# felipefelixarias/a2cat-vn-pytorch

Hardware: AMD Instinct MI355X
Metric: env-steps/sec (whole node), 4096 parallel cached-THOR envs at 1/2/4/8 GPUs (higher is better)
Workload: dtype u8; 1 GPU; cached-THOR VectorEnv.step, 20 synthetic 24x24 scenes (626 MB frame cache, HBM-resident), 4096 envs/GPU, 84x84x3 frames, uniform random actions, auto-reset, TimeLimit 900; envs_per_gpu=4096, scenes=20, parallelism=dp1 (independent env shards, replicated scene cache)

## Files before the change

a2cat-vn-pytorch_amd/csrc/vn_policy.hip:

```cpp
#include <hip/hip_runtime.h>

#include <algorithm>
#include <cstdio>
#include <cstdlib>
#include <mutex>
#include <new>
#include <map>
#include <tuple>
#include <unordered_map>

#include "vn_common.h"
#include "vn_gemm.h"
#include "vn_lstm.h"
#include "vn_aux.h"
#include "vn_unreal.h"
#include "vn_skinny.h"

#include "vn_frames.h"
#include "vn_conv1.h"
namespace vn {

template <int H, int W, int OH, int OW>
struct FramesIm2col {
  FrameSrc src;
// ... 932 lines not shown
  DgradA<COUT, 4, 2, OH, OW, HYC, WXC> fa{dz, M};
  DgradB<COUT, 4, 2, CINF> fb{WT, cin, g * cin, PY, PX};
  EpiMaskParity<H, W, 2, PY, PX, HYC, WXC> ep{out, X, g, G, cin};
  launch_gemm_x6<128, 32, 32, 4, 1>(fa, fb, ep, M, cin, 4 * COUT, st);
}

template <int H, int OH>
constexpr int k4s2_covered() {
  return H < 2 * (OH - 1) + 4 ? H : 2 * (OH - 1) + 4;
}

template <int H, int W, int CH, int CW>
__global__ void zero_uncovered_kernel(float* __restrict__ out, int nimg_g, int cin) {
  constexpr int NU = H * W - CH * CW;
  const int64_t i = (int64_t)blockIdx.x * blockDim.x + threadIdx.x;
  const int c4n = cin / 4;
  if (i >= (int64_t)nimg_g * NU * c4n) return;
  const int c4 = (int)(i % c4n);
  const int64_t q = i / c4n;
  const int u = (int)(q % NU);
  const int64_t ng = q / NU;
  int y, x;
  if (u < (H - CH) * W) {
    y = CH + u / W;
    x = u % W;
  } else {
    const int v = u - (H - CH) * W;
    y = v / (W - CW);
    x = CW + v % (W - CW);
  }
  *reinterpret_cast<f4*>(out + ((ng * H + y) * W + x) * cin + 4 * c4) = f4zero();
}

template <int SH_, int SW_, int YC_, int XC_, int KC_, int NCOL_, int WPC_>
struct ParityDg {
  static constexpr int SH = SH_, SW = SW_, YC = YC_, XC = XC_, KC = KC_, NCOL = NCOL_, WPC = WPC_;
  static constexpr int NP = SH * SW;
  static constexpr int NPC = YC * XC;
  static constexpr int PS = KC + 8;
  static constexpr int rows(int img) { return (img * NPC + 15) / 16 * 16 + XC + 1; }
  static constexpr int IMG = NPC >= 64 ? ((size_t)3 * rows(2) * KC * 2 <= 160 * 1024 ? 2 : 1) : 64 / NPC;
  static constexpr int NR = rows(IMG);
  static constexpr int NTL = NCOL / (16 * WPC);
  static constexpr int KS = KC / 32;
  static constexpr int NT = 256 * WPC;
  static constexpr size_t LDS = (size_t)3 * NR * KC * 2;
  static constexpr bool fits = LDS <= 160 * 1024;
  static_assert(KC % 32 == 0 && NCOL % (16 * WPC) == 0, "k steps of 32, whole 16-column tiles per wave");
  static_assert(KC == 32 || KC == 64, "plane rows of 4 or 8 quads (dg_quad_off)");
  static_assert(XC == SW + 1 && YC == SH + 1, "k4 s2 classes: the map plus one gap row and column");
};

template <class S, class EP>
__global__ __launch_bounds__(S::NT, S::NT >= 512 ? 1 : 2) void parity_dgrad_x6_kernel(const float* __restrict__ map,
                                                                const float* __restrict__ WT, EP ep, int n) {
  constexpr int SW = S::SW, XC = S::XC, KC = S::KC, NCOL = S::NCOL, WPC = S::WPC;
  constexpr int NP = S::NP, NPC = S::NPC, IMG = S::IMG, NTL = S::NTL, KS = S::KS, NT = S::NT;
  constexpr int ROWS = IMG * NP, PL = S::NR * KC, C4 = KC / 4, NQ = KC / 8;
  constexpr int TILES = (IMG * NPC + 15) / 16, NZ = (ROWS * C4 + NT - 1) / NT;
  extern __shared__ __attribute__((aligned(16))) uint8_t smem_pdg[];
  uint16_t* zs = reinterpret_cast<uint16_t*>(smem_pdg);
  const int tid = threadIdx.x, lane = tid & 63;
  const int wave = __builtin_amdgcn_readfirstlane(tid >> 6);
  const int cls = wave / WPC, py = cls >> 1, px = cls & 1;
  const int col0 = (wave % WPC) * NTL * 16;
  const int i16 = lane & 15, q = lane >> 4;
  bf16x8_t bw[4][KS][NTL][3];
#pragma unroll
  for (int t = 0; t < 4; ++t) {
    const int ky = py + 2 * (t >> 1), kx = px + 2 * (t & 1);
#pragma unroll
    for (int h = 0; h < KS; ++h)
#pragma unroll
      for (int nt = 0; nt < NTL; ++nt) {
        union { uint16_t u[8]; bf16x8_t v; } b0, b1, b2;
        const float* w = WT + ((int64_t)(ky * 4 + kx) * NCOL + col0 + 16 * nt + i16) * KC + 32 * h + 8 * q;
#pragma unroll
        for (int j = 0; j < 8; ++j) split3_bf16(w[j], b0.u[j], b1.u[j], b2.u[j]);
        bw[t][h][nt][0] = b0.v;
        bw[t][h][nt][1] = b1.v;
        bw[t][h][nt][2] = b2.v;
      }
  }
  for (int i = tid; i < 3 * PL / 8; i += NT) reinterpret_cast<uint4*>(zs)[i] = uint4{0u, 0u, 0u, 0u};
  __syncthreads();
  const int items = (n + IMG - 1) / IMG;
  f4 zr[NZ];
  auto load_z = [&](int it) {
    const int64_t r0 = (int64_t)it * ROWS, rend = (int64_t)n * NP;
    const f4* z4 = reinterpret_cast<const f4*>(map);
#pragma unroll
    for (int j = 0; j < NZ; ++j) {
      const int i = tid + j * NT;
      if (i < ROWS * C4) zr[j] = r0 + i / C4 < rend ? z4[(r0 + i / C4) * C4 + i % C4] : f4zero();
    }
  };
  constexpr bool PF = NZ <= 3;
  if (PF && (int)blockIdx.x < items) load_z(blockIdx.x);
  for (int it = blockIdx.x; it < items; it += gridDim.x) {
    if constexpr (!PF) load_z(it);
#pragma unroll
    for (int j = 0; j < NZ; ++j) {
      const int i = tid + j * NT;
      if (i < ROWS * C4) {
        uint2 t0, t1, t2;
        split3_pack(zr[j], t0, t1, t2);
        const int pix = i / C4, c = i - (i / C4) * C4, im = pix / NP, rem = pix - (pix / NP) * NP;
        const int row = im * NPC + (rem / SW + 1) * XC + rem % SW + 1;
        uint16_t* d = zs + dg_quad_off<NQ>(row, c >> 1) + 4 * (c & 1);
// ... 32 lines not shown
            c = __builtin_amdgcn_mfma_f32_16x16x32_bf16(bw[tap][h][nt][2], a[0], c, 0, 0, 0);
            c = __builtin_amdgcn_mfma_f32_16x16x32_bf16(bw[tap][h][nt][1], a[1], c, 0, 0, 0);
            c = __builtin_amdgcn_mfma_f32_16x16x32_bf16(bw[tap][h][nt][0], a[1], c, 0, 0, 0);
            c = __builtin_amdgcn_mfma_f32_16x16x32_bf16(bw[tap][h][nt][1], a[0], c, 0, 0, 0);
            c = __builtin_amdgcn_mfma_f32_16x16x32_bf16(bw[tap][h][nt][0], a[0], c, 0, 0, 0);
            acc[nt] = c;
          }
        }
      if (live) {
        const int y = 2 * yy + py, x = 2 * xx + px;
        f4 pre[NTL];
#pragma unroll
        for (int nt = 0; nt < NTL; ++nt) pre[nt] = ep.pre(img0 + im, y, x, col0 + 16 * nt + 4 * q);
#pragma unroll
        for (int nt = 0; nt < NTL; ++nt) ep.post(img0 + im, y, x, col0 + 16 * nt + 4 * q, acc[nt], pre[nt]);
      }
    }
    __syncthreads();
  }
}

template <class S, int BY>
constexpr int parity_band_nr() {
  return (BY * S::XC + 15) / 16 * 16 + S::XC + 1;
}
template <class S, int BY>
constexpr size_t parity_band_lds() {
  return (size_t)3 * parity_band_nr<S, BY>() * S::KC * 2;
}

template <class S, int BY, class EP>
__global__ __launch_bounds__(S::NT, 1) void parity_dgrad_band_x6_kernel(const float* __restrict__ map,
                                                                       const float* __restrict__ WT, EP ep, int n) {
  constexpr int SH = S::SH, SW = S::SW, YC = S::YC, XC = S::XC, KC = S::KC, NCOL = S::NCOL, WPC = S::WPC;
  constexpr int NTL = S::NTL, KS = S::KS, NT = S::NT, NQ = KC / 8;
  constexpr int NB = (YC + BY - 1) / BY;
  constexpr int ROWS = (BY + 1) * SW, PL = parity_band_nr<S, BY>() * KC, C4 = KC / 4;
  constexpr int TILES = (BY * XC + 15) / 16, NZ = (ROWS * C4 + NT - 1) / NT;
  extern __shared__ __attribute__((aligned(16))) uint8_t smem_pdb[];
  uint16_t* zs = reinterpret_cast<uint16_t*>(smem_pdb);
  const int tid = threadIdx.x, lane = tid & 63;
  const int wave = __builtin_amdgcn_readfirstlane(tid >> 6);
  const int cls = wave / WPC, py = cls >> 1, px = cls & 1;
  const int col0 = (wave % WPC) * NTL * 16;
  const int i16 = lane & 15, q = lane >> 4;
  bf16x8_t bw[4][KS][NTL][3];
#pragma unroll
  for (int t = 0; t < 4; ++t) {
    const int ky = py + 2 * (t >> 1), kx = px + 2 * (t & 1);
#pragma unroll
    for (int h = 0; h < KS; ++h)
#pragma unroll
      for (int nt = 0; nt < NTL; ++nt) {
        union { uint16_t u[8]; bf16x8_t v; } b0, b1, b2;
        const float* w = WT + ((int64_t)(ky * 4 + kx) * NCOL + col0 + 16 * nt + i16) * KC + 32 * h + 8 * q;
#pragma unroll
        for (int j = 0; j < 8; ++j) split3_bf16(w[j], b0.u[j], b1.u[j], b2.u[j]);
        bw[t][h][nt][0] = b0.v;
        bw[t][h][nt][1] = b1.v;
        bw[t][h][nt][2] = b2.v;
      }
  }
  for (int i = tid; i < 3 * PL / 8; i += NT) reinterpret_cast<uint4*>(zs)[i] = uint4{0u, 0u, 0u, 0u};
  __syncthreads();
  const int items = n * NB;
  for (int it = blockIdx.x; it < items; it += gridDim.x) {
    const int img = it / NB, y0 = (it - (it / NB) * NB) * BY;
    {
      const f4* z4 = reinterpret_cast<const f4*>(map) + (int64_t)img * SH * SW * C4;
#pragma unroll 2
      for (int j = 0; j < NZ; ++j) {
        const int i = tid + j * NT;
        if (i < ROWS * C4) {
          const int rp = i / C4, c = i - (i / C4) * C4;
          const int oy = y0 - 1 + rp / SW;
          const f4 v = (oy >= 0 && oy < SH) ? z4[((int64_t)oy * SW + rp % SW) * C4 + c] : f4zero();
          uint2 t0, t1, t2;
          split3_pack(v, t0, t1, t2);
          uint16_t* d = zs + dg_quad_off<NQ>((rp / SW) * XC + rp % SW + 1, c >> 1) + 4 * (c & 1);
          *reinterpret_cast<uint2*>(d) = t0;
          *reinterpret_cast<uint2*>(d + PL) = t1;
          *reinterpret_cast<uint2*>(d + 2 * PL) = t2;
        }
      }
    }
    __syncthreads();
#pragma unroll 1
    for (int tile = 0; tile < TILES; ++tile) {
// ... 24 lines not shown
            c = __builtin_amdgcn_mfma_f32_16x16x32_bf16(bw[tap][h][nt][1], a[0], c, 0, 0, 0);
            c = __builtin_amdgcn_mfma_f32_16x16x32_bf16(bw[tap][h][nt][0], a[0], c, 0, 0, 0);
            acc[nt] = c;
          }
        }
      if (live) {
        const int y = 2 * yy + py, x = 2 * xx + px;
        f4 pre[NTL];
#pragma unroll
        for (int nt = 0; nt < NTL; ++nt) pre[nt] = ep.pre(img, y, x, col0 + 16 * nt + 4 * q);
#pragma unroll
        for (int nt = 0; nt < NTL; ++nt) ep.post(img, y, x, col0 + 16 * nt + 4 * q, acc[nt], pre[nt]);
      }
    }
    __syncthreads();
  }
}

template <class S>
constexpr int parity_band_rows() {
  int bmax = 0;
  for (int b = S::YC; b >= 1 && bmax == 0; --b)
    if ((size_t)3 * ((b * S::XC + 15) / 16 * 16 + S::XC + 1) * S::KC * 2 <= 150 * 1024) bmax = b;
  if (bmax == 0) return 0;
  const int nb = (S::YC + bmax - 1) / bmax;
  return (S::YC + nb - 1) / nb;
}

template <int IH, int IW>
struct EpiDgMaskG2 {
  const float* X;
  float* out;
  int mask_goal = 1;
  __device__ __forceinline__ int64_t index(int img, int y, int x, int col) const {
    return ((((int64_t)img * 2 + (col >> 5)) * IH + y) * IW + x) * 32 + (col & 31);
  }
  __device__ __forceinline__ f4 pre(int img, int y, int x, int col) const {
    return *reinterpret_cast<const f4*>(X + index(img, y, x, col));
  }
  __device__ __forceinline__ void post(int img, int y, int x, int col, f4 v, f4 xm) const {
    const bool m = mask_goal || col < 32;
#pragma unroll
    for (int e = 0; e < 4; ++e) v[e] = (!m || xm[e] > 0.0f) ? v[e] : 0.0f;
    *reinterpret_cast<f4*>(out + index(img, y, x, col)) = v;
  }
};

__global__ __launch_bounds__(256) void goal_dz2_reduce_kernel(float* __restrict__ dz2, const float* __restrict__ X2,
                                                              int64_t frame_f4, const int32_t* __restrict__ list,
                                                              const int32_t* __restrict__ count,
                                                              const int32_t* __restrict__ run_length, int E) {
  const int64_t total = (int64_t)(*count) * frame_f4;
  for (int64_t idx = (int64_t)blockIdx.x * 256 + threadIdx.x; idx < total; idx += (int64_t)gridDim.x * 256) {
    const int64_t j = idx / frame_f4, c = idx - j * frame_f4;
    const int64_t r = list[j];
    const int len = run_length[r];
    f4* d = reinterpret_cast<f4*>(dz2) + (2 * r + 1) * frame_f4 + c;
    f4 acc = *d;
    for (int i = 1; i < len; ++i) acc += reinterpret_cast<const f4*>(dz2)[(2 * (r + (int64_t)i * E) + 1) * frame_f4 + c];
    const f4 x = reinterpret_cast<const f4*>(X2)[(2 * r + 1) * frame_f4 + c];
#pragma unroll
    for (int e = 0; e < 4; ++e) acc[e] = x[e] > 0.0f ? acc[e] : 0.0f;
    *d = acc;
  }
}

template <int OH, int OW, int C>
struct EpiDgBias {
  float* out;
  const float* bias;
  int relu;
  __device__ __forceinline__ f4 pre(int, int, int, int col) const {
    return *reinterpret_cast<const f4*>(bias + col);
  }
  __device__ __forceinline__ void post(int img, int y, int x, int col, f4 v, f4 b) const {
#pragma unroll
    for (int e = 0; e < 4; ++e) v[e] = relu ? fmaxf(v[e] + b[e], 0.0f) : v[e] + b[e];
    *reinterpret_cast<f4*>(out + (((int64_t)img * OH + y) * OW + x) * C + col) = v;
  }
};

template <class S, class EP>
inline int launch_parity_dgrad_x6(const float* map, const float* WT, EP ep, int n, hipStream_t st) {
  const void* kfn = (const void*)parity_dgrad_x6_kernel<S, EP>;
  VN_HIP(ensure_dyn_lds(kfn, S::LDS));
  const int items = (n + S::IMG - 1) / S::IMG;
  const int blocks = std::min(items, resident_blocks(kfn, S::NT, S::LDS));
  if (blocks > 0) hipLaunchKernelGGL((parity_dgrad_x6_kernel<S, EP>), dim3(blocks), dim3(S::NT), S::LDS, st, map, WT, ep, n);
  return VN_OK;
}

template <int IH_, int IW_, int OH_, int OW_, int CO_, int G_, int BR_, int IMG_, int CX_ = 32, bool BIAS_ = true>
struct WgSpec {
  static constexpr int IH = IH_, IW = IW_, OH = OH_, OW = OW_, CO = CO_, G = G_, BR = BR_, IMG = IMG_;
  static constexpr int CX = CX_;
  static constexpr bool BIAS = BIAS_;
  static constexpr int NTW = CX / 16;
  static constexpr int NB = OH / BR;
  static constexpr int XR = 2 * BR + 2 < IH ? 2 * BR + 2 : IH;
  static constexpr int NPX = XR * IW;
  static constexpr int KP = IMG * BR * OW, KSTEPS = (KP + 31) / 32;
  static constexpr bool KPERM = CX == 32;
  static constexpr int PZ = CO + (KPERM ? 16 : 8), PX = CX + 8;
  static constexpr int RZ = KP + 1, RX = IMG * NPX + 1;
  static constexpr size_t LDS = (size_t)3 * (RZ * PZ + RX * PX) * 2;
  static constexpr bool fits = OH % BR == 0 && LDS <= 160 * 1024;
  static constexpr int KW = 16 * G * CX;
  static constexpr int SLAB_N = KW + (BIAS ? 1 : 0);
  static constexpr int MT = CO / 16, C4 = CO / 4;
};

__device__ __forceinline__ s16x4_ lds_tr(const uint16_t* p) {
  typedef __attribute__((address_space(3))) s16x4_ lds_s16x4;
  return __builtin_amdgcn_ds_read_tr16_b64_v4i16((lds_s16x4*)(p));
}

template <int Q, int RSTRIDE, int ROWS>
__device__ __forceinline__ void wg_slot(int i, int& row, int& c) {
  constexpr int D = (Q == 8 && RSTRIDE % 32 == 20) ? 4 : (Q == 8 && RSTRIDE % 32 == 24) ? 2 : 0;
  c = i % Q;
  const int t = i / Q;
  if constexpr (D > 0) {
    constexpr int FULL = ROWS / (2 * D) * (2 * D);
    const int m = t % (2 * D);
    row = t < FULL ? t - m + (m >> 1) + (m & 1) * D : t;
  } else {
    row = t;
  }
}

template <class S>
__global__ __launch_bounds__(512, 1) void conv_wgrad_x6_kernel(const float* __restrict__ dZ, const float* __restrict__ X,
                                                            float* __restrict__ slab, int n, FrameList fl,
                                                            const int32_t* __restrict__ gdelta) {
  constexpr int IH = S::IH, IW = S::IW, OH = S::OH, OW = S::OW, CO = S::CO, G = S::G, BR = S::BR, IMG = S::IMG;
  constexpr int NPX = S::NPX, KP = S::KP, PZ = S::PZ, PX = S::PX, MT = S::MT, C4 = S::C4;
  constexpr int CX = S::CX, X4 = CX / 4, NTW = S::NTW, NTT = 2 * NTW;
  constexpr int PLZ = S::RZ * PZ, PLX = S::RX * PX, NT = 512, BP = BR * OW;
  constexpr int NZ = (KP * C4 + NT - 1) / NT, NX = (IMG * NPX * X4 + NT - 1) / NT;
  static_assert(NT % C4 == 0, "a thread's dZ channel quad is fixed");
  extern __shared__ __attribute__((aligned(16))) uint8_t smem_wg[];
  uint16_t* zs = reinterpret_cast<uint16_t*>(smem_wg);
  uint16_t* xs = zs + 3 * PLZ;
  float* red = reinterpret_cast<float*>(smem_wg);
  const int g = blockIdx.y;
  const int tid = threadIdx.x, lane = tid & 63;
  const int wave = __builtin_amdgcn_readfirstlane(tid >> 6);
  const int Gq = lane >> 4, q = (lane >> 2) & 3, p = lane & 3;
  for (int i = tid; i < 3 * (PZ + PX) / 2; i += NT) {
    const int pl = i / ((PZ + PX) / 2), e = i - pl * ((PZ + PX) / 2);
    if (e < PZ / 2)
      reinterpret_cast<uint32_t*>(zs + pl * PLZ + KP * PZ)[e] = 0u;
    else
      reinterpret_cast<uint32_t*>(xs + pl * PLX + IMG * NPX * PX)[e - PZ / 2] = 0u;
  }
  f4 acc[MT][NTT];
#pragma unroll
  for (int mt = 0; mt < MT; ++mt)
#pragma unroll
    for (int nt = 0; nt < NTT; ++nt) acc[mt][nt] = f4zero();
  f4 dbs = f4zero();
  n = fl_count(fl, n);
  const int items = (n + IMG - 1) / IMG * S::NB;
  f4 zr[NZ], xr[NX];
  auto load = [&](int it) {
    const int img0 = (it / S::NB) * IMG, band = it - (it / S::NB) * S::NB;
    int zi[IMG], xi[IMG];
#pragma unroll
    for (int im = 0; im < IMG; ++im) {
      zi[im] = fl_frame(fl, min(img0 + im, n - 1));
      xi[im] = zi[im] + ((gdelta && g == 1) ? fl_sload(gdelta + zi[im]) : 0);
    }
#pragma unroll
    for (int j = 0; j < NZ; ++j) {
      int k, c;
      wg_slot<C4, PZ / 2, KP>(min(tid + j * NT, KP * C4 - 1), k, c);
      const int im = k / BP;
      int imc = zi[0];
#pragma unroll
      for (int m = 1; m < IMG; ++m) imc = im == m ? zi[m] : imc;
      zr[j] = reinterpret_cast<const f4*>(dZ)[(((int64_t)imc * OH + band * BR) * OW + (k - im * BP)) * C4 + c];
    }
#pragma unroll
    for (int j = 0; j < NX; ++j) {
      int r, c;
      wg_slot<X4, PX / 2, IMG * NPX>(min(tid + j * NT, IMG * NPX * X4 - 1), r, c);
      const int im = r / NPX;
      int imc = xi[0];
#pragma unroll
      for (int m = 1; m < IMG; ++m) imc = im == m ? xi[m] : imc;
      xr[j] = reinterpret_cast<const f4*>(X)[((((int64_t)imc * G + g) * IH + 2 * band * BR) * IW + (r - im * NPX)) * X4 + c];
    }
  };
  if ((int)blockIdx.x < items) load(blockIdx.x);
  for (int it = blockIdx.x; it < items; it += gridDim.x) {
    const int img0 = (it / S::NB) * IMG;
#pragma unroll
    for (int j = 0; j < NZ; ++j) {
      const int i = tid + j * NT;
      if (i < KP * C4) {
        int k, c;
        wg_slot<C4, PZ / 2, KP>(i, k, c);
        const f4 z = img0 + k / BP < n ? zr[j] : f4zero();
        if (S::BIAS && g == 0) dbs += z;
// ... 95 lines not shown
      const int c4 = tid >> 2, e = tid & 3;
      float s = 0.0f;
      for (int k = 0; k < NT / C4; ++k) s += red[4 * (c4 + C4 * k) + e];
      row[(int64_t)(4 * c4 + e) * S::SLAB_N + S::SLAB_N - 1] = s;
    }
  }
}

template <class S>
inline int launch_conv_wgrad_x6(const float* dz, const float* X, int n, float* slab, int64_t slab_cap, float* dW,
                                float* db, hipStream_t st, FrameList fl = FrameList{}, const int32_t* gdelta = nullptr) {
  const void* kfn = (const void*)conv_wgrad_x6_kernel<S>;
  VN_HIP(ensure_dyn_lds(kfn, S::LDS));
  const int items = (n + S::IMG - 1) / S::IMG * S::NB;
  constexpr int kParts = 32;
  const int64_t nel = (int64_t)S::CO * S::SLAB_N;
  int bx = std::max(1, std::min(items, resident_blocks(kfn, 512, S::LDS) / S::G));
  bx = (int)std::max<int64_t>(1, std::min<int64_t>(bx, slab_cap / nel - kParts));
  hipLaunchKernelGGL((conv_wgrad_x6_kernel<S>), dim3(bx, S::G), dim3(512), S::LDS, st, dz, X, slab, n, fl, gdelta);
  const float* src = slab;
  int nsrc = bx;
  if (bx >= 2 * kParts) {
    float* part = slab + (int64_t)bx * nel;
    hipLaunchKernelGGL(slab_partial_kernel, dim3((unsigned)((nel + 255) / 256), kParts), dim3(256), 0, st, slab, bx, nel,
                       part);
    src = part;
    nsrc = kParts;
  }
  hipLaunchKernelGGL(wgrad_reduce_kernel, dim3((unsigned)((nel + 255) / 256)), dim3(256), 0, st, src, nsrc, S::CO,
                     S::SLAB_N, S::KW, dW, S::BIAS ? db : nullptr, nullptr);
  return VN_OK;
}

template <int IH, int IW, int OH, int OW>
using Conv3WgWhole = WgSpec<IH, IW, OH, OW, 64, 2, OH, (OH * OW >= 32 ? 1 : 32 / (OH * OW))>;
template <int IH, int IW, int OH, int OW>
using Conv3Wg = std::conditional_t<Conv3WgWhole<IH, IW, OH, OW>::fits, Conv3WgWhole<IH, IW, OH, OW>,
                                   WgSpec<IH, IW, OH, OW, 64, 2, 1, 2>>;
template <int IH, int IW, int OH, int OW>
using Conv2WgWide = WgSpec<IH, IW, OH, OW, 32, 1, (OH % 4 == 0 && OH > 9 ? 4 : OH), 1>;
template <int IH, int IW, int OH, int OW>
using Conv2Wg = std::conditional_t<Conv2WgWide<IH, IW, OH, OW>::fits, Conv2WgWide<IH, IW, OH, OW>,
                                   WgSpec<IH, IW, OH, OW, 32, 1, 1, 1>>;

template <int COUT, int CIN, int H, int W, int OH, int OW, int PY, int PX>
inline void dgrad_class_groups(const float* dz, const float* WT, float* out, const float* X, int nimg, int G,
                               hipStream_t st, int mask_goal = 1) {
  constexpr int CH = k4s2_covered<H, OH>(), CW = k4s2_covered<W, OW>();
  constexpr int HYC = (CH - PY + 1) / 2, WXC = (CW - PX + 1) / 2;
  const int M = nimg * HYC * WXC;
  DgradA<COUT, 4, 2, OH, OW, HYC, WXC> fa{dz, M};
  static_assert(CIN == 32, "conv3: two groups of 32 channels (W^T rows of 64)");
  DgradB<COUT, 4, 2, 2 * CIN> fb{WT, G * CIN, 0, PY, PX};
  EpiMaskParityG<H, W, 2, PY, PX, HYC, WXC, CIN> ep{out, X, G, mask_goal};
  launch_gemm_x6<128, 64, 32, 2, 2>(fa, fb, ep, M, G * CIN, 4 * COUT, st);
}

template <int COUT, int CIN, int H, int W, int OH, int OW>
inline int dgrad_all_classes_groups(const float* dz, const float* WT, float* out, const float* X, int nimg, int G,
                                     hipStream_t st, int mask_goal = 1) {
  constexpr int CH = k4s2_covered<H, OH>(), CW = k4s2_covered<W, OW>();
  using S = ParityDg<OH, OW, CH / 2, CW / 2, COUT, 2 * CIN, 2>;
  const bool generic = getenv("VN_DGRAD_GENERIC") != nullptr;
  constexpr int BY = parity_band_rows<S>();
  if (CH % 2 == 0 && CW % 2 == 0 && S::fits && COUT == 64 && CIN == 32 && G == 2 && !generic) {
    if constexpr (CH % 2 == 0 && CW % 2 == 0 && S::fits) {
      const int rc = launch_parity_dgrad_x6<S>(dz, WT, EpiDgMaskG2<H, W>{X, out, mask_goal}, nimg, st);
      if (rc != VN_OK) return rc;
    }
  } else if (CH % 2 == 0 && CW % 2 == 0 && !S::fits && BY > 0 && COUT == 64 && CIN == 32 && G == 2 && !generic) {
    if constexpr (CH % 2 == 0 && CW % 2 == 0 && !S::fits && BY > 0) {
      const void* kfn = (const void*)parity_dgrad_band_x6_kernel<S, BY, EpiDgMaskG2<H, W>>;
      constexpr size_t lds = parity_band_lds<S, BY>();
      VN_HIP(ensure_dyn_lds(kfn, lds));
      const int items = nimg * ((S::YC + BY - 1) / BY);
      const int blocks = std::min(items, resident_blocks(kfn, S::NT, lds));
      if (blocks > 0)
        hipLaunchKernelGGL((parity_dgrad_band_x6_kernel<S, BY, EpiDgMaskG2<H, W>>), dim3(blocks), dim3(S::NT), lds, st,
                           dz, WT, EpiDgMaskG2<H, W>{X, out, mask_goal}, nimg);
    }
  } else {
    dgrad_class_groups<COUT, CIN, H, W, OH, OW, 0, 0>(dz, WT, out, X, nimg, G, st, mask_goal);
    dgrad_class_groups<COUT, CIN, H, W, OH, OW, 0, 1>(dz, WT, out, X, nimg, G, st, mask_goal);
    dgrad_class_groups<COUT, CIN, H, W, OH, OW, 1, 0>(dz, WT, out, X, nimg, G, st, mask_goal);
    dgrad_class_groups<COUT, CIN, H, W, OH, OW, 1, 1>(dz, WT, out, X, nimg, G, st, mask_goal);
  }
  if constexpr (CH < H || CW < W) {
    const int64_t total = (int64_t)nimg * G * (H * W - CH * CW) * (CIN / 4);
    hipLaunchKernelGGL((zero_uncovered_kernel<H, W, CH, CW>), dim3((unsigned)((total + 255) / 256)), dim3(256), 0, st,
                       out, nimg * G, CIN);
  }
  return VN_OK;
}

template <int COUT, int CINF, int H, int W, int OH, int OW>
inline void dgrad_all_classes(const float* dz, const float* WT, float* out, const float* X, int nimg, int g, int G,
                              int cin, hipStream_t st) {
  dgrad_class<COUT, CINF, H, W, OH, OW, 0, 0>(dz, WT, out, X, nimg, g, G, cin, st);
  dgrad_class<COUT, CINF, H, W, OH, OW, 0, 1>(dz, WT, out, X, nimg, g, G, cin, st);
  dgrad_class<COUT, CINF, H, W, OH, OW, 1, 0>(dz, WT, out, X, nimg, g, G, cin, st);
  dgrad_class<COUT, CINF, H, W, OH, OW, 1, 1>(dz, WT, out, X, nimg, g, G, cin, st);
}

template <int H0, int W0>
constexpr bool kConv1LdsFrame = (size_t)H0 * W0 * 3 <= 96 * 1024;

template <int H0, int W0>
struct Geo {
  static constexpr int OH1 = (H0 - 7) / 4 + 1, OW1 = (W0 - 7) / 4 + 1;
  static constexpr int OH2 = (OH1 - 4) / 2 + 1, OW2 = (OW1 - 4) / 2 + 1;
  static constexpr int OH3 = (OH2 - 4) / 2 + 1, OW3 = (OW2 - 4) / 2 + 1;
  static constexpr int FCIN = 32 * OH3 * OW3;
};

struct Acts {
  float* X[5];
  uint32_t* M1;
  int64_t off;
};

inline Acts acts_at(const PolicyLayout& L, float* base, int64_t cap, int64_t off) {
  Acts a;
  a.off = off;
// ... 161 lines not shown
    DenseRows fb{P + L.l[3].w, 64, 32};
    EpiBiasAct ep{a.X[3], 32, P + L.l[3].b, 1};
    launch_gemm_x6<128, 32, 32, 4, 1>(fa, fb, ep, fa.M, 32, 64, st);
  }
  {
    EpiBiasAct ep{a.X[4], 512, P + L.l[4].b, 1};
    if (n <= kSkinnyRows) {
      launch_skinny(a.X[3], G::FCIN, P + L.l[4].w, G::FCIN, ep, n, 512, G::FCIN, st);
    } else {
      DenseRows fa{a.X[3], G::FCIN, n};
      DenseRows fb{P + L.l[4].w, G::FCIN, 512};
      launch_gemm_x6_sk<64, 64, 32, 2, 2, 64>(fa, fb, ep, n, 512, G::FCIN, st, L);
    }
  }
  if (out) {
    EpiBiasAct ep{out, OUT_LD, P + L.l[5].b, 0};
    if (n <= kSkinnyRows) {
      launch_skinny(a.X[4], 512, P + L.l[5].w, 512, ep, n, A1, 512, st);
    } else {
      DenseRows fa{a.X[4], 512, n};
      DenseRows fb{P + L.l[5].w, 512, A1};
      launch_gemm_sk<64, 16, 32, 4, 1>(fa, fb, ep, n, A1, 512, st, L);
    }
  }
  VN_HIP(hipGetLastError());
  return VN_OK;
}

struct BwdWork {
  float* wt;
  float* dz5;
  float* dz4;
  float* dz3;
  float* dz2;
  float* slab;
  int64_t slab_cap;
};

inline int64_t slab_floats(const PolicyLayout& L) {
  return 24ll << 20;
}

inline int64_t workspace_floats(const PolicyLayout& L, int64_t n) {
  return L.wt_total + n * 512 + n * L.FCIN + n * L.sz[2] + n * L.sz[1] + slab_floats(L) + 64;
}

inline BwdWork carve(const PolicyLayout& L, float* ws, int64_t n) {
  BwdWork w;
  float* p = ws;
  w.wt = p;
  p += L.wt_total;
  w.dz5 = p;
  p += n * 512;
  w.dz4 = p;
  p += n * L.FCIN;
  w.dz3 = p;
  p += n * L.sz[2];
  w.dz2 = p;
  p += n * L.sz[1];
  w.slab = p;
  w.slab_cap = slab_floats(L);
  return w;
}

template <int H0, int W0>
int backward_impl(const PolicyLayout& L, const float* P, const FrameSrc& src, int n, const Acts& a,
                  const float* dout, const float* dz5_in, const float* dx4_extra, float* Gr, const BwdWork& w,
                  hipStream_t st, const vn_goal_runs* gr = nullptr) {
  using G = Geo<H0, W0>;
  const int A1 = L.A + 1;
  const FrameList fl = gr ? FrameList{gr->goal_list, gr->goal_count, n} : FrameList{};
  auto T = [&](int i) { return w.wt + L.wt_off[i]; };
  const float* dz5 = dz5_in ? dz5_in : w.dz5;
  {
    TransposeSet ts;
    for (int i = 1; i < 6; ++i) ts.add(P + L.l[i].w, L.l[i].cout, L.l[i].kp, T(i));
    launch_transpose_set(ts, st);
  }
  const int n9 = n * G::OH3 * G::OW3;
  if (!dz5_in) {
    DenseRows fa{dout, OUT_LD, n};
    DenseRows fb{T(5), A1, 512};
    EpiMask ep{w.dz5, a.X[4], 512};
    launch_gemm<64, 64, 32, 2, 2>(fa, fb, ep, n, 512, A1, st);
    Im2colT<DenseRows> fbw{DenseRows{a.X[4], 512, n}, 512};
    launch_wgrad<32, 64, 2, 2>(dout, OUT_LD, A1, fbw, 512, n, w.slab, w.slab_cap, Gr + L.l[5].w, Gr + L.l[5].b, st);
  }
  {
    DenseRows fa{dz5, 512, n};
    DenseRows fb{T(4), 512, G::FCIN};
    const bool big = G::FCIN >= 1024 && n >= 256;
    auto dgrad = [&](auto ep) {
      if (big)
        launch_gemm_x6<128, 128, 32, 2, 2>(fa, fb, ep, n, G::FCIN, 512, st);
      else
        launch_gemm_x6_sk<64, 64, 32, 2, 2>(fa, fb, ep, n, G::FCIN, 512, st, L);
    };
    if (dx4_extra)
      dgrad(EpiMaskAdd{w.dz4, a.X[3], G::FCIN, dx4_extra});
    else
      dgrad(EpiMask{w.dz4, a.X[3], G::FCIN});
    Im2colT<DenseRows> fbw{DenseRows{a.X[3], G::FCIN, n}, G::FCIN};
    launch_wgrad6<128, 128, 2, 2>(dz5, 512, 512, fbw, G::FCIN, n, w.slab, w.slab_cap, Gr + L.l[4].w, Gr + L.l[4].b,
                                  st);
  }
  {
    DenseRows fa{w.dz4, 32, n9};
    DenseRows fb{T(3), 32, 64};
    EpiMask ep{w.dz3, a.X[2], 64};
    launch_gemm_x6<64, 64, 32, 2, 2>(fa, fb, ep, n9, 64, 32, st);
    Im2colT<DenseRows> fbw{DenseRows{a.X[2], 64, n9}, 64};
    launch_wgrad<32, 64, 2, 2>(w.dz4, 32, 32, fbw, 64, n9, w.slab, w.slab_cap, Gr + L.l[3].w, Gr + L.l[3].b, st);
  }
  {
    using Im = NhwcIm2col<32, 4, 4, 2, G::OH2, G::OW2, G::OH3, G::OW3, 2>;
    Im2colT<Im> fbw{Im{a.X[1], n9}, 1024};
    using Wg = Conv3Wg<G::OH2, G::OW2, G::OH3, G::OW3>;
    if (Wg::fits && !getenv("VN_WGRAD_GENERIC")) {
      if constexpr (Wg::fits) {
        const int rc = launch_conv_wgrad_x6<Wg>(w.dz3, a.X[1], n, w.slab, w.slab_cap, Gr + L.l[2].w, Gr + L.l[2].b, st,
                                                FrameList{}, gr ? gr->goal_delta : nullptr);
        if (rc != VN_OK) return rc;
      }
    } else if (gr) {
      if constexpr (kGoalRunsGeo<H0, W0>) {
        using ImG = NhwcIm2colGoal<32, 4, 4, 2, G::OH2, G::OW2, G::OH3, G::OW3>;
        Im2colT<ImG> fbg{ImG{a.X[1], n9, gr->goal_delta}, 1024};
        launch_wgrad6<64, 128, 2, 2>(w.dz3, 64, 64, fbg, 1024, n9, w.slab, w.slab_cap, Gr + L.l[2].w, Gr + L.l[2].b,
                                     st);
      }
    } else {
      launch_wgrad6<64, 128, 2, 2>(w.dz3, 64, 64, fbw, 1024, n9, w.slab, w.slab_cap, Gr + L.l[2].w, Gr + L.l[2].b, st);
    }
    const int rc =
        dgrad_all_classes_groups<64, 32, G::OH2, G::OW2, G::OH3, G::OW3>(w.dz3, T(2), w.dz2, a.X[1], n, 2, st, gr ? 0 : 1);
    if (rc != VN_OK) return rc;
    if (gr) {
      constexpr int64_t frame_f4 = (int64_t)G::OH2 * G::OW2 * 8;
      const int blocks = (int)std::min<int64_t>((n * frame_f4 + 255) / 256, 4096);
      hipLaunchKernelGGL(goal_dz2_reduce_kernel, dim3(blocks), dim3(256), 0, st, w.dz2, a.X[1], frame_f4, gr->goal_list,
                         gr->goal_count, gr->run_length, gr->num_envs);
    }
  }
  {
    const int frames = 2 * n;
    using Bd2 = Conv2WgBand<G::OH1, G::OW1, G::OH2, G::OW2>;
    const int blocks = std::min(frames * Bd2::NB, kConv2WgradBlocks);
    constexpr size_t lds = conv2_wgrad_lds<G::OH1, G::OW1, G::OH2, G::OW2>();
    using Wg2 = Conv2Wg<G::OH1, G::OW1, G::OH2, G::OW2>;
    if (Wg2::fits && !getenv("VN_WGRAD_GENERIC") && !getenv("VN_CONV2WG_F32")) {
      if constexpr (Wg2::fits) {
        const int rc = launch_conv_wgrad_x6<Wg2>(w.dz2, a.X[0], frames, w.slab, w.slab_cap, Gr + L.l[1].w, Gr + L.l[1].b,
                                                 st, fl);
        if (rc != VN_OK) return rc;
      }
    } else if constexpr (lds <= 80 * 1024) {
      VN_HIP(ensure_dyn_lds((const void*)conv2_wgrad_kernel<G::OH1, G::OW1, G::OH2, G::OW2>, lds));
      float* bias_slab = w.slab + (int64_t)blocks * 32 * 512;
      hipLaunchKernelGGL((conv2_wgrad_kernel<G::OH1, G::OW1, G::OH2, G::OW2>), dim3(blocks), dim3(256), lds, st,
                         a.X[0], w.dz2, frames, w.slab, bias_slab, fl);
      constexpr int kParts = 32;
      float* part = bias_slab + (int64_t)blocks * 32;
      float* bpart = part + (int64_t)kParts * 32 * 512;
      hipLaunchKernelGGL(slab_partial_kernel, dim3((32 * 512 + 255) / 256, kParts), dim3(256), 0, st, w.slab, blocks,
                         (int64_t)32 * 512, part);
      hipLaunchKernelGGL(slab_partial_kernel, dim3(1, kParts), dim3(32), 0, st, bias_slab, blocks, (int64_t)32, bpart);
      hipLaunchKernelGGL(sum_slabs_kernel, dim3((32 * 512 + 255) / 256), dim3(256), 0, st, part, kParts,
                         (int64_t)32 * 512, Gr + L.l[1].w);
      hipLaunchKernelGGL(sum_slabs_kernel, dim3(1), dim3(32), 0, st, bpart, kParts, (int64_t)32, Gr + L.l[1].b);
    } else {
      using Im = NhwcIm2col<32, 4, 4, 2, G::OH1, G::OW1, G::OH2, G::OW2, 1>;
      const int P2 = 2 * n * G::OH2 * G::OW2;
      Im2colT<Im> fbw{Im{a.X[0], P2}, 512};
      launch_wgrad<32, 64, 2, 2>(w.dz2, 32, 32, fbw, 512, P2, w.slab, w.slab_cap, Gr + L.l[1].w, Gr + L.l[1].b, st);
// ... 1256 lines not shown
```

Before: 150.1 million env-steps/s.

## Compute conv3 goal-branch backward once per goal run instead of per sample

Adds a runs-based conv3 backward path. Goal-group dz3 gradients are first summed over each goal run. Weight-gradient and data-gradient kernels for the goal half then process one item per run rather than every sample. This removes the separate per-sample goal dz2 reduction and avoids redundant work on repeated goal frames, at the cost of an extra dz3g buffer and more kernel launches. Whether this path affects the env-steps metric depends on whether the training backward pass is part of the timed loop.

```diff
diff --git a/a2cat-vn-pytorch_amd/csrc/vn_policy.hip b/a2cat-vn-pytorch_amd/csrc/vn_policy.hip
--- a/a2cat-vn-pytorch_amd/csrc/vn_policy.hip
+++ b/a2cat-vn-pytorch_amd/csrc/vn_policy.hip
@@ -988,9 +988,10 @@
   *reinterpret_cast<f4*>(out + ((ng * H + y) * W + x) * cin + 4 * c4) = f4zero();
 }
 
-template <int SH_, int SW_, int YC_, int XC_, int KC_, int NCOL_, int WPC_>
+template <int SH_, int SW_, int YC_, int XC_, int KC_, int NCOL_, int WPC_, int WLD_ = NCOL_>
 struct ParityDg {
   static constexpr int SH = SH_, SW = SW_, YC = YC_, XC = XC_, KC = KC_, NCOL = NCOL_, WPC = WPC_;
+  static constexpr int WLD = WLD_;
   static constexpr int NP = SH * SW;
   static constexpr int NPC = YC * XC;
   static constexpr int PS = KC + 8;
@@ -1010,7 +1011,7 @@
 template <class S, class EP>
 __global__ __launch_bounds__(S::NT, S::NT >= 512 ? 1 : 2) void parity_dgrad_x6_kernel(const float* __restrict__ map,
                                                                 const float* __restrict__ WT, EP ep, int n) {
-  constexpr int SW = S::SW, XC = S::XC, KC = S::KC, NCOL = S::NCOL, WPC = S::WPC;
+  constexpr int SW = S::SW, XC = S::XC, KC = S::KC, WPC = S::WPC;
   constexpr int NP = S::NP, NPC = S::NPC, IMG = S::IMG, NTL = S::NTL, KS = S::KS, NT = S::NT;
   constexpr int ROWS = IMG * NP, PL = S::NR * KC, C4 = KC / 4, NQ = KC / 8;
   constexpr int TILES = (IMG * NPC + 15) / 16, NZ = (ROWS * C4 + NT - 1) / NT;
@@ -1021,6 +1022,7 @@
   const int cls = wave / WPC, py = cls >> 1, px = cls & 1;
   const int col0 = (wave % WPC) * NTL * 16;
   const int i16 = lane & 15, q = lane >> 4;
+  n = ep.items(n);
   bf16x8_t bw[4][KS][NTL][3];
 #pragma unroll
   for (int t = 0; t < 4; ++t) {
@@ -1030,7 +1032,7 @@
 #pragma unroll
       for (int nt = 0; nt < NTL; ++nt) {
         union { uint16_t u[8]; bf16x8_t v; } b0, b1, b2;
-        const float* w = WT + ((int64_t)(ky * 4 + kx) * NCOL + col0 + 16 * nt + i16) * KC + 32 * h + 8 * q;
+        const float* w = WT + ((int64_t)(ky * 4 + kx) * S::WLD + col0 + 16 * nt + i16) * KC + 32 * h + 8 * q;
 #pragma unroll
         for (int j = 0; j < 8; ++j) split3_bf16(w[j], b0.u[j], b1.u[j], b2.u[j]);
         bw[t][h][nt][0] = b0.v;
@@ -1129,7 +1131,7 @@
 template <class S, int BY, class EP>
 __global__ __launch_bounds__(S::NT, 1) void parity_dgrad_band_x6_kernel(const float* __restrict__ map,
                                                                        const float* __restrict__ WT, EP ep, int n) {
-  constexpr int SH = S::SH, SW = S::SW, YC = S::YC, XC = S::XC, KC = S::KC, NCOL = S::NCOL, WPC = S::WPC;
+  constexpr int SH = S::SH, SW = S::SW, YC = S::YC, XC = S::XC, KC = S::KC, WPC = S::WPC;
   constexpr int NTL = S::NTL, KS = S::KS, NT = S::NT, NQ = KC / 8;
   constexpr int NB = (YC + BY - 1) / BY;
   constexpr int ROWS = (BY + 1) * SW, PL = parity_band_nr<S, BY>() * KC, C4 = KC / 4;
@@ -1141,6 +1143,7 @@
   const int cls = wave / WPC, py = cls >> 1, px = cls & 1;
   const int col0 = (wave % WPC) * NTL * 16;
   const int i16 = lane & 15, q = lane >> 4;
+  n = ep.items(n);
   bf16x8_t bw[4][KS][NTL][3];
 #pragma unroll
   for (int t = 0; t < 4; ++t) {
@@ -1150,7 +1153,7 @@
 #pragma unroll
       for (int nt = 0; nt < NTL; ++nt) {
         union { uint16_t u[8]; bf16x8_t v; } b0, b1, b2;
-        const float* w = WT + ((int64_t)(ky * 4 + kx) * NCOL + col0 + 16 * nt + i16) * KC + 32 * h + 8 * q;
+        const float* w = WT + ((int64_t)(ky * 4 + kx) * S::WLD + col0 + 16 * nt + i16) * KC + 32 * h + 8 * q;
 #pragma unroll
         for (int j = 0; j < 8; ++j) split3_bf16(w[j], b0.u[j], b1.u[j], b2.u[j]);
         bw[t][h][nt][0] = b0.v;
@@ -1241,6 +1244,7 @@
   const float* X;
   float* out;
   int mask_goal = 1;
+  __device__ __forceinline__ int items(int n) const { return n; }
   __device__ __forceinline__ int64_t index(int img, int y, int x, int col) const {
     return ((((int64_t)img * 2 + (col >> 5)) * IH + y) * IW + x) * 32 + (col & 31);
   }
@@ -1274,11 +1278,65 @@
   }
 }
 
+__global__ __launch_bounds__(256) void goal_dz3_sum_kernel(const float* __restrict__ dz3, float* __restrict__ dz3g,
+                                                           int64_t map_f4, const int32_t* __restrict__ list,
+                                                           const int32_t* __restrict__ count,
+                                                           const int32_t* __restrict__ run_length, int E) {
+  const int64_t total = (int64_t)(*count) * map_f4;
+  for (int64_t idx = (int64_t)blockIdx.x * 256 + threadIdx.x; idx < total; idx += (int64_t)gridDim.x * 256) {
+    const int64_t j = idx / map_f4, c = idx - j * map_f4;
+    const int64_t r = list[j];
+    const int len = run_length[r];
+    f4 acc = reinterpret_cast<const f4*>(dz3)[r * map_f4 + c];
+    for (int i = 1; i < len; ++i) acc += reinterpret_cast<const f4*>(dz3)[(r + (int64_t)i * E) * map_f4 + c];
+    reinterpret_cast<f4*>(dz3g)[idx] = acc;
+  }
+}
+
+template <int IH, int IW>
+struct EpiDgImageG {
+  const float* X;
+  float* out;
+  __device__ __forceinline__ int items(int n) const { return n; }
+  __device__ __forceinline__ int64_t index(int img, int y, int x, int col) const {
+    return (((int64_t)img * 2 * IH + y) * IW + x) * 32 + col;
+  }
+  __device__ __forceinline__ f4 pre(int img, int y, int x, int col) const {
+    return *reinterpret_cast<const f4*>(X + index(img, y, x, col));
+  }
+  __device__ __forceinline__ void post(int img, int y, int x, int col, f4 v, f4 xm) const {
+#pragma unroll
+    for (int e = 0; e < 4; ++e) v[e] = xm[e] > 0.0f ? v[e] : 0.0f;
+    *reinterpret_cast<f4*>(out + index(img, y, x, col)) = v;
+  }
+};
+
+template <int IH, int IW>
+struct EpiDgGoalRun {
+  const float* X;
+  float* out;
+  const int32_t* __restrict__ list;
+  const int32_t* count;
+  __device__ __forceinline__ int items(int n) const { return min(n, fl_sload(count)); }
+  __device__ __forceinline__ int64_t index(int run, int y, int x, int col) const {
+    return ((((int64_t)list[run] * 2 + 1) * IH + y) * IW + x) * 32 + col;
+  }
+  __device__ __forceinline__ f4 pre(int run, int y, int x, int col) const {
+    return *reinterpret_cast<const f4*>(X + index(run, y, x, col));
+  }
+  __device__ __forceinline__ void post(int run, int y, int x, int col, f4 v, f4 xm) const {
+#pragma unroll
+    for (int e = 0; e < 4; ++e) v[e] = xm[e] > 0.0f ? v[e] : 0.0f;
+    *reinterpret_cast<f4*>(out + index(run, y, x, col)) = v;
+  }
+};
+
 template <int OH, int OW, int C>
 struct EpiDgBias {
   float* out;
   const float* bias;
   int relu;
+  __device__ __forceinline__ int items(int n) const { return n; }
   __device__ __forceinline__ f4 pre(int, int, int, int col) const {
     return *reinterpret_cast<const f4*>(bias + col);
   }
@@ -1338,7 +1396,7 @@
   }
 }
 
-template <class S>
+template <class S, bool RUNS = false>
 __global__ __launch_bounds__(512, 1) void conv_wgrad_x6_kernel(const float* __restrict__ dZ, const float* __restrict__ X,
                                                             float* __restrict__ slab, int n, FrameList fl,
                                                             const int32_t* __restrict__ gdelta) {
@@ -1352,7 +1410,7 @@
   uint16_t* zs = reinterpret_cast<uint16_t*>(smem_wg);
   uint16_t* xs = zs + 3 * PLZ;
   float* red = reinterpret_cast<float*>(smem_wg);
-  const int g = blockIdx.y;
+  const int g = RUNS ? 1 : blockIdx.y;
   const int tid = threadIdx.x, lane = tid & 63;
   const int wave = __builtin_amdgcn_readfirstlane(tid >> 6);
   const int Gq = lane >> 4, q = (lane >> 2) & 3, p = lane & 3;
@@ -1369,7 +1427,7 @@
 #pragma unroll
     for (int nt = 0; nt < NTT; ++nt) acc[mt][nt] = f4zero();
   f4 dbs = f4zero();
-  n = fl_count(fl, n);
+  n = RUNS ? min(n, fl_sload(fl.count)) : fl_count(fl, n);
   const int items = (n + IMG - 1) / IMG * S::NB;
   f4 zr[NZ], xr[NX];
   auto load = [&](int it) {
@@ -1377,8 +1435,13 @@
     int zi[IMG], xi[IMG];
 #pragma unroll
     for (int im = 0; im < IMG; ++im) {
-      zi[im] = fl_frame(fl, min(img0 + im, n - 1));
-      xi[im] = zi[im] + ((gdelta && g == 1) ? fl_sload(gdelta + zi[im]) : 0);
+      if constexpr (RUNS) {
+        zi[im] = __builtin_amdgcn_readfirstlane(min(img0 + im, n - 1));
+        xi[im] = fl_sload(fl.goals + zi[im]);
+      } else {
+        zi[im] = fl_frame(fl, min(img0 + im, n - 1));
+        xi[im] = zi[im] + ((gdelta && g == 1) ? fl_sload(gdelta + zi[im]) : 0);
+      }
     }
 #pragma unroll
     for (int j = 0; j < NZ; ++j) {
@@ -1540,6 +1603,37 @@
   return VN_OK;
 }
 
+template <class S>
+inline int launch_conv3_wgrad_runs(const float* dz, const float* dzg, const float* X, int n, float* slab,
+                                   int64_t slab_cap, float* dW, float* db, hipStream_t st, const int32_t* goal_list,
+                                   const int32_t* goal_count) {
+  static_assert(S::G == 2 && S::BIAS, "conv3: image and goal group, bias with the image group");
+  const void* kfn = (const void*)conv_wgrad_x6_kernel<S>;
+  const void* kfr = (const void*)conv_wgrad_x6_kernel<S, true>;
+  VN_HIP(ensure_dyn_lds(kfn, S::LDS));
+  VN_HIP(ensure_dyn_lds(kfr, S::LDS));
+  const int items = (n + S::IMG - 1) / S::IMG * S::NB;
+  constexpr int kParts = 32;
+  const int64_t nel = (int64_t)S::CO * S::SLAB_N;
+  int bx = std::max(1, std::min({items, resident_blocks(kfn, 512, S::LDS), resident_blocks(kfr, 512, S::LDS)}));
+  bx = (int)std::max<int64_t>(1, std::min<int64_t>(bx, slab_cap / nel - kParts));
+  hipLaunchKernelGGL((conv_wgrad_x6_kernel<S>), dim3(bx, 1), dim3(512), S::LDS, st, dz, X, slab, n, FrameList{}, nullptr);
+  hipLaunchKernelGGL((conv_wgrad_x6_kernel<S, true>), dim3(bx, 1), dim3(512), S::LDS, st, dzg, X, slab, n,
+                     FrameList{goal_list, goal_count, 0}, nullptr);
+  const float* src = slab;
+  int nsrc = bx;
+  if (bx >= 2 * kParts) {
+    float* part = slab + (int64_t)bx * nel;
+    hipLaunchKernelGGL(slab_partial_kernel, dim3((unsigned)((nel + 255) / 256), kParts), dim3(256), 0, st, slab, bx, nel,
+                       part);
+    src = part;
+    nsrc = kParts;
+  }
+  hipLaunchKernelGGL(wgrad_reduce_kernel, dim3((unsigned)((nel + 255) / 256)), dim3(256), 0, st, src, nsrc, S::CO,
+                     S::SLAB_N, S::KW, dW, db, nullptr);
+  return VN_OK;
+}
+
 template <int IH, int IW, int OH, int OW>
 using Conv3WgWhole = WgSpec<IH, IW, OH, OW, 64, 2, OH, (OH * OW >= 32 ? 1 : 32 / (OH * OW))>;
 template <int IH, int IW, int OH, int OW>
@@ -1597,6 +1691,52 @@
     const int64_t total = (int64_t)nimg * G * (H * W - CH * CW) * (CIN / 4);
     hipLaunchKernelGGL((zero_uncovered_kernel<H, W, CH, CW>), dim3((unsigned)((total + 255) / 256)), dim3(256), 0, st,
                        out, nimg * G, CIN);
+  }
+  return VN_OK;
+}
+
+template <int H, int W, int OH, int OW>
+constexpr bool conv3_dgrad_runs_fits() {
+  constexpr int CH = k4s2_covered<H, OH>(), CW = k4s2_covered<W, OW>();
+  if constexpr (CH % 2 == 0 && CW % 2 == 0) {
+    using S = ParityDg<OH, OW, CH / 2, CW / 2, 64, 32, 1, 64>;
+    return S::fits || parity_band_rows<S>() > 0;
+  }
+  return false;
+}
+
+template <class S, class EP>
+inline int launch_parity_dgrad_any(const float* map, const float* WT, EP ep, int n, hipStream_t st) {
+  if constexpr (S::fits) {
+    return launch_parity_dgrad_x6<S>(map, WT, ep, n, st);
+  } else {
+    constexpr int BY = parity_band_rows<S>();
+    const void* kfn = (const void*)parity_dgrad_band_x6_kernel<S, BY, EP>;
+    constexpr size_t lds = parity_band_lds<S, BY>();
+    VN_HIP(ensure_dyn_lds(kfn, lds));
+    const int items = n * ((S::YC + BY - 1) / BY);
+    const int blocks = std::min(items, resident_blocks(kfn, S::NT, lds));
+    if (blocks > 0)
+      hipLaunchKernelGGL((parity_dgrad_band_x6_kernel<S, BY, EP>), dim3(blocks), dim3(S::NT), lds, st, map, WT, ep, n);
+    return VN_OK;
+  }
+}
+
+template <int WPC, int H, int W, int OH, int OW>
+inline int conv3_dgrad_runs(const float* dz, const float* dzg, const float* WT, float* out, const float* X, int n,
+                            const int32_t* goal_list, const int32_t* goal_count, hipStream_t st) {
+  constexpr int CH = k4s2_covered<H, OH>(), CW = k4s2_covered<W, OW>();
+  if constexpr (conv3_dgrad_runs_fits<H, W, OH, OW>()) {
+    using S = ParityDg<OH, OW, CH / 2, CW / 2, 64, 32, WPC, 64>;
+    int rc = launch_parity_dgrad_any<S>(dz, WT, EpiDgImageG<H, W>{X, out}, n, st);
+    if (rc != VN_OK) return rc;
+    rc = launch_parity_dgrad_any<S>(dzg, WT + 32 * 64, EpiDgGoalRun<H, W>{X, out, goal_list, goal_count}, n, st);
+    if (rc != VN_OK) return rc;
+    if constexpr (CH < H || CW < W) {
+      const int64_t total = (int64_t)n * 2 * (H * W - CH * CW) * 8;
+      hipLaunchKernelGGL((zero_uncovered_kernel<H, W, CH, CW>), dim3((unsigned)((total + 255) / 256)), dim3(256), 0, st,
+                         out, n * 2, 32);
+    }
   }
   return VN_OK;
 }
@@ -1824,6 +1964,7 @@
   float* dz5;
   float* dz4;
   float* dz3;
+  float* dz3g;
   float* dz2;
   float* slab;
   int64_t slab_cap;
@@ -1834,7 +1975,7 @@
 }
 
 inline int64_t workspace_floats(const PolicyLayout& L, int64_t n) {
-  return L.wt_total + n * 512 + n * L.FCIN + n * L.sz[2] + n * L.sz[1] + slab_floats(L) + 64;
+  return L.wt_total + n * 512 + n * L.FCIN + 2 * n * L.sz[2] + n * L.sz[1] + slab_floats(L) + 64;
 }
 
 inline BwdWork carve(const PolicyLayout& L, float* ws, int64_t n) {
@@ -1847,6 +1988,8 @@
   w.dz4 = p;
   p += n * L.FCIN;
   w.dz3 = p;
+  p += n * L.sz[2];
+  w.dz3g = p;
   p += n * L.sz[2];
   w.dz2 = p;
   p += n * L.sz[1];
@@ -1908,30 +2051,52 @@
     using Im = NhwcIm2col<32, 4, 4, 2, G::OH2, G::OW2, G::OH3, G::OW3, 2>;
     Im2colT<Im> fbw{Im{a.X[1], n9}, 1024};
     using Wg = Conv3Wg<G::OH2, G::OW2, G::OH3, G::OW3>;
-    if (Wg::fits && !getenv("VN_WGRAD_GENERIC")) {
-      if constexpr (Wg::fits) {
-        const int rc = launch_conv_wgrad_x6<Wg>(w.dz3, a.X[1], n, w.slab, w.slab_cap, Gr + L.l[2].w, Gr + L.l[2].b, st,
-                                                FrameList{}, gr ? gr->goal_delta : nullptr);
+    constexpr bool kRunsForm = kGoalRunsGeo<H0, W0> && Wg::fits && conv3_dgrad_runs_fits<G::OH2, G::OW2, G::OH3, G::OW3>();
+    if (kRunsForm && gr && !getenv("VN_WGRAD_GENERIC") && !getenv("VN_DGRAD_GENERIC") &&
+        !getenv("VN_CONV3_BWD_PER_SAMPLE")) {
+      if constexpr (kRunsForm) {
+        constexpr int64_t map_f4 = (int64_t)G::OH3 * G::OW3 * 16;
+        const int blocks = (int)std::min<int64_t>((n * map_f4 + 255) / 256, 4096);
+        hipLaunchKernelGGL(goal_dz3_sum_kernel, dim3(blocks), dim3(256), 0, st, w.dz3, w.dz3g, map_f4, gr->goal_list,
+                           gr->goal_count, gr->run_length, gr->num_envs);
+        int rc = launch_conv3_wgrad_runs<Wg>(w.dz3, w.dz3g, a.X[1], n, w.slab, w.slab_cap, Gr + L.l[2].w, Gr + L.l[2].b,
+                                             st, gr->goal_list, gr->goal_count);
+        if (rc != VN_OK) return rc;
+        constexpr bool kSmallMaps = G::OH3 * G::OW3 < 32;
+        const char* ov = getenv("VN_CONV3DG_WPC");
+        const int wpc = ov && (ov[0] == '1' || ov[0] == '2') ? ov[0] - '0' : (kSmallMaps ? 1 : 2);
+        rc = wpc == 1 ? conv3_dgrad_runs<1, G::OH2, G::OW2, G::OH3, G::OW3>(w.dz3, w.dz3g, T(2), w.dz2, a.X[1], n,
+                                                                           gr->goal_list, gr->goal_count, st)
+                      : conv3_dgrad_runs<2, G::OH2, G::OW2, G::OH3, G::OW3>(w.dz3, w.dz3g, T(2), w.dz2, a.X[1], n,
+                                                                           gr->goal_list, gr->goal_count, st);
         if (rc != VN_OK) return rc;
       }
-    } else if (gr) {
-      if constexpr (kGoalRunsGeo<H0, W0>) {
-        using ImG = NhwcIm2colGoal<32, 4, 4, 2, G::OH2, G::OW2, G::OH3, G::OW3>;
-        Im2colT<ImG> fbg{ImG{a.X[1], n9, gr->goal_delta}, 1024};
-        launch_wgrad6<64, 128, 2, 2>(w.dz3, 64, 64, fbg, 1024, n9, w.slab, w.slab_cap, Gr + L.l[2].w, Gr + L.l[2].b,
-                                     st);
+    } else {
+      if (Wg::fits && !getenv("VN_WGRAD_GENERIC")) {
+        if constexpr (Wg::fits) {
+          const int rc = launch_conv_wgrad_x6<Wg>(w.dz3, a.X[1], n, w.slab, w.slab_cap, Gr + L.l[2].w, Gr + L.l[2].b, st,
+                                                  FrameList{}, gr ? gr->goal_delta : nullptr);
+          if (rc != VN_OK) return rc;
+        }
+      } else if (gr) {
+        if constexpr (kGoalRunsGeo<H0, W0>) {
+          using ImG = NhwcIm2colGoal<32, 4, 4, 2, G::OH2, G::OW2, G::OH3, G::OW3>;
+          Im2colT<ImG> fbg{ImG{a.X[1], n9, gr->goal_delta}, 1024};
+          launch_wgrad6<64, 128, 2, 2>(w.dz3, 64, 64, fbg, 1024, n9, w.slab, w.slab_cap, Gr + L.l[2].w, Gr + L.l[2].b,
+                                       st);
+        }
+      } else {
+        launch_wgrad6<64, 128, 2, 2>(w.dz3, 64, 64, fbw, 1024, n9, w.slab, w.slab_cap, Gr + L.l[2].w, Gr + L.l[2].b, st);
       }
-    } else {
-      launch_wgrad6<64, 128, 2, 2>(w.dz3, 64, 64, fbw, 1024, n9, w.slab, w.slab_cap, Gr + L.l[2].w, Gr + L.l[2].b, st);
-    }
-    const int rc =
-        dgrad_all_classes_groups<64, 32, G::OH2, G::OW2, G::OH3, G::OW3>(w.dz3, T(2), w.dz2, a.X[1], n, 2, st, gr ? 0 : 1);
-    if (rc != VN_OK) return rc;
-    if (gr) {
-      constexpr int64_t frame_f4 = (int64_t)G::OH2 * G::OW2 * 8;
-      const int blocks = (int)std::min<int64_t>((n * frame_f4 + 255) / 256, 4096);
-      hipLaunchKernelGGL(goal_dz2_reduce_kernel, dim3(blocks), dim3(256), 0, st, w.dz2, a.X[1], frame_f4, gr->goal_list,
-                         gr->goal_count, gr->run_length, gr->num_envs);
+      const int rc =
+          dgrad_all_classes_groups<64, 32, G::OH2, G::OW2, G::OH3, G::OW3>(w.dz3, T(2), w.dz2, a.X[1], n, 2, st, gr ? 0 : 1);
+      if (rc != VN_OK) return rc;
+      if (gr) {
+        constexpr int64_t frame_f4 = (int64_t)G::OH2 * G::OW2 * 8;
+        const int blocks = (int)std::min<int64_t>((n * frame_f4 + 255) / 256, 4096);
+        hipLaunchKernelGGL(goal_dz2_reduce_kernel, dim3(blocks), dim3(256), 0, st, w.dz2, a.X[1], frame_f4, gr->goal_list,
+                           gr->goal_count, gr->run_length, gr->num_envs);
+      }
     }
   }
   {
```

After: 146.1 million env-steps/s. -2.6%, worse.
